# SciML/SciMLSensitivity.jl

Hardware: NVIDIA H100
Metric: ensemble adjoint trajectories/sec (higher is better)
Workload: dtype f64

## Files before the change

include/b200adj.h:

```cpp
#ifndef B200ADJ_H
#define B200ADJ_H
#include <stdint.h>
#ifdef __cplusplus
extern "C" {
#endif

enum {
    B200ADJ_FAM_LV = 0,
    B200ADJ_FAM_LORENZ = 1,
    B200ADJ_FAM_ROBERTSON = 2,
    B200ADJ_FAM_SDE_LV = 3,
    B200ADJ_FAM_MLP = 4,
    B200ADJ_FAM_SDE_LINEAR = 5,
    B200ADJ_FAM_BALL = 6,
    B200ADJ_FAM_RELAX = 7
};
#define B200ADJ_FAM_USER_BASE 100
int32_t b200adj_register_family(const char* plugin_path, int32_t* family_id);
int32_t b200adj_family_info(int32_t family_id, int32_t* d, int32_t* P, const char** name);

enum { B200ADJ_SA_INTERPOLATING = 0, B200ADJ_SA_GAUSS = 1, B200ADJ_SA_QUADRATURE = 2, B200ADJ_SA_BACKSOLVE = 3,
       B200ADJ_SA_GAUSSKRONROD = 4  };
enum { B200ADJ_ST_TSIT5_FIXED = 0, B200ADJ_ST_ROSENBROCK23 = 1, B200ADJ_ST_EM = 2, B200ADJ_ST_EULER_HEUN = 3,
       B200ADJ_ST_TSIT5_ADAPTIVE = 4  };
enum { B200ADJ_F64 = 0, B200ADJ_F32 = 1, B200ADJ_BF16_F32ACC = 2 };
enum { B200ADJ_COST_EXPLICIT = 0, B200ADJ_COST_AFFINE = 1 };

#define B200ADJ_FLAG_NO_START            1u
#define B200ADJ_FLAG_NO_CHECKPOINTING    2u
#define B200ADJ_FLAG_CKPT_EVERY_STEP     4u
#define B200ADJ_FLAG_STORED_NOISE        8u

#define B200ADJ_FLAG_TRACE              16u
#define B200ADJ_FLAG_NO_ROTATE          32u
#define B200ADJ_FLAG_DENSE_FORWARD      64u
#define B200ADJ_FLAG_NCCL_ALLREDUCE    128u
#define B200ADJ_CREATE_FLAGS (B200ADJ_FLAG_STORED_NOISE | B200ADJ_FLAG_TRACE | B200ADJ_FLAG_NO_ROTATE | B200ADJ_FLAG_DENSE_FORWARD | B200ADJ_FLAG_NCCL_ALLREDUCE)

#define B200ADJ_OK                 0
#define B200ADJ_ERR_INVALID       -1
#define B200ADJ_ERR_UNSUPPORTED   -2
#define B200ADJ_ERR_NO_DEVICE     -3
#define B200ADJ_ERR_CUDA          -4
#define B200ADJ_ERR_STATE         -5
#define B200ADJ_ERR_OOM           -6

typedef struct b200adj_cfg {
    int32_t rhs_family, sensealg, stepper, dtype;
    int32_t d, P, m, K;
    int64_t N;
    double  t0, t1, dt;
    double  abstol, reltol;
// ... 74 lines not shown
```

scimlsensitivity.jl_b200/_lib.py:

```python
import ctypes as C
import os
import shutil
import subprocess

_PKG = os.path.dirname(os.path.abspath(__file__))
_ROOT = os.path.dirname(_PKG)
_CSRC = os.path.join(_PKG, "csrc")
LIB_PATH = os.environ.get("B200ADJ_LIB", os.path.join(_PKG, "libb200adj.so"))

FAM = {"lv": 0, "lorenz": 1, "robertson": 2, "sde_lv": 3, "mlp": 4, "sde_linear": 5, "ball": 6, "relax": 7}
SA = {"interpolating": 0, "gauss": 1, "quadrature": 2, "backsolve": 3, "gauss_kronrod": 4}
ST = {"tsit5_fixed": 0, "rosenbrock23": 1, "em": 2, "euler_heun": 3, "tsit5_adaptive": 4}
DTYPE = {"f64": 0, "f32": 1, "bf16_f32acc": 2}
COST = {"explicit": 0, "affine": 1}
FLAG_NO_START, FLAG_NO_CHECKPOINTING, FLAG_CKPT_EVERY_STEP, FLAG_STORED_NOISE, FLAG_TRACE, FLAG_NO_ROTATE, FLAG_DENSE_FORWARD, FLAG_NCCL_ALLREDUCE = 1, 2, 4, 8, 16, 32, 64, 128
ERR = {0: "OK", -1: "INVALID", -2: "UNSUPPORTED", -3: "NO_DEVICE", -4: "CUDA", -5: "STATE", -6: "OOM"}

EXPORTS = ["b200adj_create", "b200adj_forward", "b200adj_reverse", "b200adj_set_reverse_options", "b200adj_set_tolerances", "b200adj_set_continuous_cost", "b200adj_set_cost_family", "b200adj_register_family", "b200adj_family_info", "b200adj_set_events", "b200adj_set_event_param_shift", "b200adj_set_continuous_callback", "b200adj_set_continuous_callback_params", "b200adj_event_times", "b200adj_family_conditions", "b200adj_set_family_events", "b200adj_event_flags", "b200adj_get_noise", "b200adj_set_stream",
           "b200adj_synchronize", "b200adj_launch_count", "b200adj_get_step_counts", "b200adj_get_block_trace", "b200adj_destroy",
           "b200adj_last_error", "b200adj_version", "b200adj_sizeof_cfg",
           "b200adj_comm_unique_id", "b200adj_comm_init", "b200adj_comm_init_all", "b200adj_comm_allreduce", "b200adj_comm_size", "b200adj_comm_is_fused"]


class B200AdjError(RuntimeError):
    def __init__(self, code, msg):
        super().__init__(f"b200adj error {code} ({ERR.get(code, '?')}): {msg}")
        self.code = code


class Cfg(C.Structure):
# ... 339 lines not shown
```

scimlsensitivity.jl_b200/csrc/api.cu:

```cuda
#include <dlfcn.h>

#include "handle.h"

using namespace b200adj;
namespace {

thread_local std::string g_create_error;

const double TSIT5_A[7][6] = {
    {0},
    {0.161},
    {-0.008480655492356989, 0.335480655492357},
    {2.8971530571054935, -6.359448489975075, 4.3622954328695815},
    {5.325864828439257, -11.748883564062828, 7.4955393428898365, -0.09249506636175525},
    {5.86145544294642, -12.92096931784711, 8.159367898576159, -0.071584973281401, -0.028269050394068383},
    {0.09646076681806523, 0.01, 0.4798896504144996, 1.379008574103742, -3.290069515436081, 2.324710524099774}};
const double TSIT5_C[7] = {0.0, 0.161, 0.327, 0.9, 0.9800255409045097, 1.0, 1.0};
const double TSIT5_BT[7] = {-0.00178001105222577714, -0.0008164344596567469, 0.007880878010261995, -0.1447110071732629,
                            0.5823571654525552, -0.45808210592918697, 0.015151515151515152};

std::vector<const FamilyVTable*>& family_registry() { static std::vector<const FamilyVTable*> r; return r; }

template <class F, bool FIXED_GRID, bool ROS, bool F32>
FamilyVTable builtin_family(const char* name) {
// ... 345 lines not shown
        if (block < 32 || block > 512 || (block % 32) != 0) { g_create_error = "block_threads must be a multiple of 32 in [32, 512]"; return B200ADJ_ERR_INVALID; }
        if (mlp) block = MLP_TB;
        if (ckpt_every > 1) {
            if (int32_t rc = support(SR_CKPT)) return rc;
            if (ckpt_every > S) ckpt_every = (int)S;
            const size_t need = (size_t)ckpt_every * d * block * esz(*cfg);
            if (need > 160 * 1024) { g_create_error = "checkpoint_every * d * block_threads * sizeof(real) exceeds 160 KB of shared memory: lower checkpoint_every or block_threads"; return B200ADJ_ERR_INVALID; }
        }
    }

    Handle* h = new Handle();
    h->cfg = *cfg; h->cfg.m = m; h->path = path;
    h->saveat.assign(cfg->saveat, cfg->saveat + cfg->K);
    h->cfg.saveat = h->saveat.data();
    h->S = (int)S; h->maxs = maxs; h->block = block; h->ckpt_every = ckpt_every;
    h->grid = (int)((cfg->N + block - 1) / block);
    h->nsm = nsm; h->qgrid = quad_grid(cfg->N, nsm);
    h->qpartials_blocks = (size_t)h->qgrid + 1;
    h->maxseg = ros ? 2 * maxs : 4096;
#define CREATE_TRY(expr)                                                                         \
    do { cudaError_t _e = (expr); if (_e != cudaSuccess) {                                       \
        g_create_error = std::string(#expr) + ": " + cudaGetErrorString(_e);                     \
        int32_t rc = (_e == cudaErrorMemoryAllocation) ? B200ADJ_ERR_OOM : B200ADJ_ERR_CUDA;     \
        free_all(h); delete h; return rc; } } while (0)
    CREATE_TRY(cudaSetDevice(cfg->device));
    CREATE_TRY(cudaStreamCreateWithFlags(&h->own_stream, cudaStreamNonBlocking));
    h->stream = h->own_stream;
    const size_t N = (size_t)cfg->N, e = esz(*cfg);
    h->fwd_K = cfg->K; h->fwd_saveat = h->saveat;
    CREATE_TRY(upload_table(&h->d_saveat, cfg->saveat, (size_t)cfg->K));
// ... 384 lines not shown
    } else if (h->path == Path::MLP) {
        rc = mlp_forward_dispatch(h, du0, dp, h->fwd_K > 0 ? dsaved : nullptr, dstatus);
    } else if (h->path == Path::FIXED && c.dtype == B200ADJ_F32) {
        OdeFwdArgsT<float> a;
        memset(&a, 0, sizeof(a));
        a.u0 = (const float*)du0; a.p = (const float*)dp; a.ckpt = (float*)h->d_ckpt; a.saved = h->fwd_K > 0 ? (float*)dsaved : nullptr;
        a.save_of_step = h->d_fwd_save_of_step; a.status = dstatus; a.N = c.N; a.Npad = h->Npad; a.S = h->S; a.ckpt_every = h->ckpt_every;
        cast_tables(h->tb, &a.tb);
        rc = launch(vt->fwd_f32, h, a);
    } else if (h->path == Path::FIXED) {
        OdeFwdArgs a;
        memset(&a, 0, sizeof(a));
        a.u0 = du0; a.p = dp; a.ckpt = h->d_ckpt; a.saved = h->fwd_K > 0 ? dsaved : nullptr; a.save_of_step = h->d_fwd_save_of_step;
        a.status = dstatus; a.N = c.N; a.Npad = h->Npad; a.S = h->S; a.tb = h->tb; a.ckpt_every = h->ckpt_every;
        a.event_of_step = h->d_event_of_step; a.ev_s = h->d_ev_s; a.ev_c = h->d_ev_c; a.ev_ps = h->d_ev_ps; a.ev_pc = h->d_ev_pc; a.nev = h->nev;
        rc = launch(vt->fwd, h, a);
    } else {
        SdeFwdArgs a;
        a.u0 = du0; a.p = dp; a.ckpt = h->d_ckpt; a.saved = h->fwd_K > 0 ? dsaved : nullptr; a.save_of_step = h->d_fwd_save_of_step;
        a.status = dstatus; a.N = c.N; a.S = h->S; a.h = c.dt; a.seed = c.seed; a.traj_offset = c.traj_offset;
        a.noise_in = nullptr; a.noise_out = nullptr;
        if (dW_in) {
            CUDA_TRY(h, cudaMemcpyAsync(h->d_noise, dW_in, (size_t)h->S * c.m * N * e,
                                        c.buffers_on_device ? cudaMemcpyDeviceToDevice : cudaMemcpyHostToDevice, h->stream));
            a.noise_in = h->d_noise; h->noise_valid = true;
        } else if (c.flags & B200ADJ_FLAG_STORED_NOISE) {
            a.noise_out = h->d_noise; h->noise_valid = true;
        } else {
            h->noise_valid = false;
        }
// ... 150 lines not shown
```

scimlsensitivity.jl_b200/csrc/disp_fixed.inc:

```
#include "handle.h"
namespace b200adj {
static int balanced_threads(const Handle* h, int slots) {
    const bool no_rotate = (h->cfg.flags & B200ADJ_FLAG_NO_ROTATE) != 0;
    if (!no_rotate && slots > 128 && (slots % 128) != 0) return ((slots + 127) / 128) * 128;
    return slots;
}
template <class Fam>
int launch_fwd(Handle* h, const OdeFwdArgs& a) {
    if (h->nev > 0) {
        if (h->cfg.shared_p) tsit5_forward_kernel<Fam, true, double, true><<<h->grid, h->block, 0, h->stream>>>(a);
        else tsit5_forward_kernel<Fam, false, double, true><<<h->grid, h->block, 0, h->stream>>>(a);
        h->launches++;
        return 0;
    }
    if (h->cfg.shared_p) tsit5_forward_kernel<Fam, true><<<h->grid, h->block, 0, h->stream>>>(a);
    else tsit5_forward_kernel<Fam, false><<<h->grid, h->block, 0, h->stream>>>(a);
    h->launches++;
    return 0;
}
template <class Fam, int SA, bool SHARED_P, int COST, bool CONT, class R>
int launch_rev_seg(Handle* h, const OdeRevArgsT<R>& a, int threads) {
    if constexpr (SA == SA_INTERP || SA == SA_GAUSS) {
        const size_t smem = rev_seg_smem_bytes<Fam::D, R>(h->block, h->ckpt_every);
        if (smem > 30 * 1024 && cudaFuncSetAttribute(tsit5_reverse_kernel<Fam, SA, SHARED_P, COST, CONT, R, true>, cudaFuncAttributeMaxDynamicSharedMemorySize, (int)smem) != cudaSuccess) return B200ADJ_ERR_CUDA;
// ... 44 lines not shown
    a.slots = h->block; a.ckpt_every = h->ckpt_every;
    const int threads = SA == SA_BACKSOLVE ? h->block : balanced_threads(h, h->block);
    if (h->ckpt_every > 1) return h->cont_on ? launch_rev_seg<Fam, SA, SHARED_P, COST, true, double>(h, a, threads)
                                             : launch_rev_seg<Fam, SA, SHARED_P, COST, false, double>(h, a, threads);
    const size_t smem = SA == SA_BACKSOLVE ? 0 : rev_smem_bytes<Fam::D>(h->block);
    if (h->nev > 0) {
        if constexpr (SA == SA_QUAD) return B200ADJ_ERR_UNSUPPORTED;
        else {
            if (h->cont_on) return B200ADJ_ERR_UNSUPPORTED;
            if (smem > 30 * 1024 && cudaFuncSetAttribute(tsit5_reverse_kernel<Fam, SA, SHARED_P, COST, false, double, false, true>, cudaFuncAttributeMaxDynamicSharedMemorySize, (int)smem) != cudaSuccess) return B200ADJ_ERR_CUDA;
            tsit5_reverse_kernel<Fam, SA, SHARED_P, COST, false, double, false, true><<<h->grid, h->block, smem, h->stream>>>(a);
            h->launches++;
            return 0;
        }
    }
    if (h->cont_on) {
        if (smem > 30 * 1024 && cudaFuncSetAttribute(tsit5_reverse_kernel<Fam, SA, SHARED_P, COST, true>, cudaFuncAttributeMaxDynamicSharedMemorySize, (int)smem) != cudaSuccess) return B200ADJ_ERR_CUDA;
        tsit5_reverse_kernel<Fam, SA, SHARED_P, COST, true><<<h->grid, threads, smem, h->stream>>>(a);
    } else {
        if (smem > 30 * 1024 && cudaFuncSetAttribute(tsit5_reverse_kernel<Fam, SA, SHARED_P, COST, false>, cudaFuncAttributeMaxDynamicSharedMemorySize, (int)smem) != cudaSuccess) return B200ADJ_ERR_CUDA;
        tsit5_reverse_kernel<Fam, SA, SHARED_P, COST, false><<<h->grid, threads, smem, h->stream>>>(a);
    }
    h->launches++;
    return 0;
}
template <class Fam, int SA>
int launch_rev_sa(Handle* h, const OdeRevArgs& a) {
    const bool sp = h->cfg.shared_p;
    const bool ex = h->cfg.cost_kind == B200ADJ_COST_EXPLICIT;
    if (sp) return ex ? launch_rev_b<Fam, SA, true, COST_EXPLICIT>(h, a) : launch_rev_b<Fam, SA, true, COST_AFFINE>(h, a);
    return ex ? launch_rev_b<Fam, SA, false, COST_EXPLICIT>(h, a) : launch_rev_b<Fam, SA, false, COST_AFFINE>(h, a);
}
template <class Fam>
int launch_rev(Handle* h, const OdeRevArgs& a) {
    switch (h->cfg.sensealg) {
    case B200ADJ_SA_INTERPOLATING: return launch_rev_sa<Fam, SA_INTERP>(h, a);
    case B200ADJ_SA_GAUSS: return launch_rev_sa<Fam, SA_GAUSS>(h, a);
    case B200ADJ_SA_BACKSOLVE: return launch_rev_sa<Fam, SA_BACKSOLVE>(h, a);
    case B200ADJ_SA_GAUSSKRONROD: return launch_rev_sa<Fam, SA_GK>(h, a);
    case B200ADJ_SA_QUADRATURE: {
        const b200adj_cfg& c = h->cfg;
        int rc = ensure_quad_buffers(h);
        if (rc) return rc;
        OdeRevArgs ar = a; ar.adj_dense = h->d_adj_dense;
        rc = launch_rev_sa<Fam, SA_QUAD>(h, ar);
        if (rc) return rc;
        Tsit5QuadArgs q;
        memset(&q, 0, sizeof(q));
        q.ckpt = h->d_ckpt; q.adj_dense = h->d_adj_dense; q.p = a.p; q.saveat = h->d_saveat;
// ... 17 lines not shown
```

scimlsensitivity.jl_b200/csrc/handle.h:

```cpp
#pragma once
#include <cuda_runtime.h>
#include <math.h>
#include <stdint.h>
#include <stdio.h>
#include <string.h>
#include <stdlib.h>

#include <string>
#include <vector>

#include "../../include/b200adj.h"
#include "ode_tsit5.cuh"
#include "sde_em.cuh"
#include "ros23.cuh"
#include "mlp.cuh"
#include "tsit5_quad.cuh"
#include "mlp_tc.cuh"
#include "mlp_tc_wide.cuh"
#include "tsit5_adaptive.cuh"

namespace b200adj {

enum class Path {
    FIXED,
    T5A,
    ROS,
    SDE,
    MLP
};

struct Handle {
    b200adj_cfg cfg;
    Path path = Path::FIXED;
    std::vector<double> saveat;
    std::vector<int32_t> save_of_step;
    int S = 0;
    int64_t Npad = 0;
    int block = 64, grid = 0, nsm = 132;
    int ckpt_every = 1;
    cudaStream_t stream = nullptr, own_stream = nullptr;
    double* d_ckpt = nullptr;
    double* d_noise = nullptr;
    double* d_partials = nullptr;
    double* d_adj_dense = nullptr;
    unsigned long long* d_trace = nullptr;
    unsigned int* d_ticket = nullptr;
    int32_t* d_save_of_step = nullptr;
    int maxs = 0;
    double adj_abstol = 0, adj_reltol = 0;
    bool cont_on = false;
    double cost_av[4] = {0, 0, 0, 0}, cost_bv[4] = {0, 0, 0, 0}, cont_av[4] = {0, 0, 0, 0}, cont_bv[4] = {0, 0, 0, 0};
    bool has_dgdp = false, has_cdgdp = false;
    double dgdp_c[8] = {0}, dgdp_e[8] = {0}, cdgdp_c[8] = {0}, cdgdp_e[8] = {0};
    float* d_kst = nullptr;
// ... 32 lines not shown
        if (_e != cudaSuccess) {                                                               \
            (h)->err = std::string(#expr) + ": " + cudaGetErrorString(_e);                     \
            return B200ADJ_ERR_CUDA;                                                           \
        }                                                                                      \
    } while (0)

inline bool is_sde(const b200adj_cfg& c) { return c.stepper == B200ADJ_ST_EM || c.stepper == B200ADJ_ST_EULER_HEUN; }
inline bool is_adaptive(const Handle* h) { return h->path == Path::T5A || h->path == Path::ROS; }
inline bool is_fixed_dt(const Handle* h) { return h->path == Path::T5A && h->cfg.stepper == B200ADJ_ST_TSIT5_FIXED; }
inline bool is_mlp_tc(const Handle* h) { return h->path == Path::MLP && h->cfg.dtype == B200ADJ_BF16_F32ACC; }
inline uint32_t kernel_flags(const Handle* h) {
    const uint32_t f = h->cfg.flags;
    return ((f & B200ADJ_FLAG_NO_START) ? KF_NO_START : 0u) | ((f & B200ADJ_FLAG_NO_CHECKPOINTING) ? KF_NO_CHECKPOINTING : 0u) |
           ((f & B200ADJ_FLAG_CKPT_EVERY_STEP) ? KF_CKPT_EVERY_STEP : 0u) | (h->cont_on ? KF_CONT_COST : 0u) |
           (is_fixed_dt(h) ? KF_FIXED_DT : 0u);
}
inline size_t esz(const b200adj_cfg& c) { return c.dtype == B200ADJ_F64 ? sizeof(double) : sizeof(float); }

void tsit5_weights(double th, double* w, double (*Rout)[4] = nullptr);
void build_tsit5_tables(double h, Tsit5Tables* t);
template <class T, class S> inline void cast_tables(const S& src, T* dst) {
    for (int i = 0; i < 7; i++) for (int j = 0; j < 6; j++) dst->hA[i][j] = (float)src.hA[i][j];
    for (int i = 0; i < 4; i++) for (int j = 0; j < 7; j++) dst->hBst[i][j] = (float)src.hBst[i][j];
    for (int i = 0; i < 3; i++) for (int j = 0; j < 7; j++) dst->hBq[i][j] = (float)src.hBq[i][j];
    for (int i = 0; i < 3; i++) dst->hGW[i] = (float)src.hGW[i];
    for (int i = 0; i < 7; i++) for (int j = 0; j < 4; j++) dst->hHm[i][j] = (float)src.hHm[i][j];
    for (int j = 0; j < 7; j++) dst->hR4[j] = (float)src.hR4[j];
}


// ... 50 lines not shown
```

scimlsensitivity.jl_b200/csrc/ode_tsit5.cuh:

```cuda
#pragma once
#include <cuda_runtime.h>
#include <stdint.h>
#include "families.cuh"
#include "quadgk.cuh"

namespace b200adj {

template <class R> struct Tsit5TablesT {
    R hA[7][6];
    R hBst[4][7];
    R hBq[3][7];
    R hGW[3];
    R hHm[7][4];
    R hR4[7];
};
using Tsit5Tables = Tsit5TablesT<double>;

constexpr int P2P_PMAX = 8, P2P_MAXRANKS = 8;
struct P2PComm {
    double* slots[P2P_MAXRANKS];
    unsigned long long* flags[P2P_MAXRANKS];
    int32_t nranks, rank;
    unsigned long long epoch;
};
// ... 90 lines not shown
        R acc = u[i];
#pragma unroll
        for (int j = 0; j < S_; j++) acc = fma(tb.hA[S_][j], k[j][i], acc);
        out[i] = acc;
    }
}
template <int D, class R> __device__ __forceinline__ void tsit5_dense(const R* u, const R (*k)[D], const R* w, R* out) {
#pragma unroll
    for (int i = 0; i < D; i++) {
        R acc = u[i];
#pragma unroll
        for (int j = 0; j < 7; j++) acc = fma(w[j], k[j][i], acc);
        out[i] = acc;
    }
}
template <int D, class R> __device__ __forceinline__ void tsit5_hermite_c4(const Tsit5TablesT<R>& tb, const R (*k)[D], R* c4) {
#pragma unroll
    for (int i = 0; i < D; i++) {
        R acc = tb.hR4[0] * k[0][i];
#pragma unroll
        for (int j = 1; j < 7; j++) acc = fma(tb.hR4[j], k[j][i], acc);
        c4[i] = acc;
    }
}
template <int D, class R>
__device__ __forceinline__ void tsit5_dense_hermite(const R* u, const R* du, const R* k1, const R* k7, const R* c4, const R* w, R* out) {
#pragma unroll
    for (int i = 0; i < D; i++) out[i] = fma(w[3], c4[i], fma(w[2], k7[i], fma(w[1], k1[i], fma(w[0], du[i], u[i]))));
}

__device__ __forceinline__ void named_bar_sync(int id, int nthreads) { asm volatile("bar.sync %0, %1;" ::"r"(id), "r"(nthreads) : "memory"); }
__device__ __forceinline__ void named_bar_arrive(int id, int nthreads) { asm volatile("bar.arrive %0, %1;" ::"r"(id), "r"(nthreads) : "memory"); }

template <int P, class R>
__device__ __forceinline__ void fixed_event_params(const double* ev_ps, const double* ev_pc, int upto, const R* p0, R* p) {
#pragma unroll
    for (int q = 0; q < P; q++) p[q] = p0[q];
    if (!ev_ps) return;
    for (int e = 0; e < upto; e++) {
#pragma unroll
        for (int q = 0; q < P; q++) p[q] = (R)ev_ps[e * P + q] * p[q] + (R)ev_pc[e * P + q];
    }
}

template <class Fam, bool SHARED_P, class R = double, bool EV = false>
__global__ void __launch_bounds__(512) tsit5_forward_kernel(const __grid_constant__ OdeFwdArgsT<R> a) {
    constexpr int D = Fam::D, P = Fam::P;
    const int64_t gi = (int64_t)blockIdx.x * blockDim.x + threadIdx.x;
    const bool active = gi < a.N;
    const int64_t i = active ? gi : a.N - 1;
    R p[P];
#pragma unroll
    for (int q = 0; q < P; q++) p[q] = SHARED_P ? __ldg(a.p + q) : __ldg(a.p + (int64_t)q * a.N + i);
    R u[D], k[7][D], tmp[D];
    load_state<D>(a.u0, a.N, i, u);
    const int64_t stride = (int64_t)D * a.N, cstride = (int64_t)D * a.Npad;
    const int CK = a.ckpt_every > 1 ? a.ckpt_every : 1;
    store_state<D>(a.ckpt, a.Npad, gi, u);
    if (active && a.saved) { int ks = a.save_of_step[0]; if (ks >= 0) store_state<D>(a.saved + (int64_t)ks * stride, a.N, i, u); }
    Fam::f(u, p, k[0]);
// ... 5 lines not shown
        tsit5_stage<D, 5>(a.tb, u, k, tmp); Fam::f(tmp, p, k[5]);
        tsit5_stage<D, 6>(a.tb, u, k, tmp);
#pragma unroll
        for (int j = 0; j < D; j++) u[j] = tmp[j];
        if (EV) {
            const int e = a.event_of_step[n + 1];
            if (e >= 0 && n + 1 < a.S) {
#pragma unroll
                for (int j = 0; j < D; j++) u[j] = (R)a.ev_s[e * D + j] * u[j] + (R)a.ev_c[e * D + j];
                if (a.ev_ps) {
#pragma unroll
                    for (int q = 0; q < P; q++) p[q] = (R)a.ev_ps[e * P + q] * p[q] + (R)a.ev_pc[e * P + q];
                }
            }
        }
        Fam::f(u, p, k[0]);
        if (CK == 1) store_state<D>(a.ckpt + (int64_t)(n + 1) * cstride, a.Npad, gi, u);
        else if ((n + 1) % CK == 0) store_state<D>(a.ckpt + (int64_t)((n + 1) / CK) * cstride, a.Npad, gi, u);
        else if (n + 1 == a.S) store_state<D>(a.ckpt + (int64_t)((a.S + CK - 1) / CK) * cstride, a.Npad, gi, u);
        if (active && a.saved) { int ks = a.save_of_step[n + 1]; if (ks >= 0) store_state<D>(a.saved + (int64_t)ks * stride, a.N, i, u); }
    }
    if (active && a.status) {
        bool ok = true;
#pragma unroll
        for (int j = 0; j < D; j++) ok = ok && isfinite(u[j]);
        a.status[i] = ok ? 0 : 1;
    }
}

__device__ __forceinline__ void st_release_sys(unsigned long long* p, unsigned long long v) { asm volatile("st.release.sys.global.u64 [%0], %1;" ::"l"(p), "l"(v) : "memory"); }
__device__ __forceinline__ unsigned long long ld_acquire_sys(const unsigned long long* p) { unsigned long long v; asm volatile("ld.acquire.sys.global.u64 %0, [%1];" : "=l"(v) : "l"(p) : "memory"); return v; }
__device__ __forceinline__ double ld_relaxed_sys_f64(const double* p) { double v; asm volatile("ld.relaxed.sys.global.f64 %0, [%1];" : "=d"(v) : "l"(p) : "memory"); return v; }

template <int P, class RO>
__device__ __forceinline__ void reduce_dp(const double* acc, double* partials, RO* dp, unsigned int* ticket, const P2PComm* pc = nullptr) {
    __shared__ double s_red[16 * P];
    const int nwarps = (int)(blockDim.x >> 5);
    __shared__ bool s_last;
    const int lane = threadIdx.x & 31, warp = threadIdx.x >> 5;
#pragma unroll
    for (int q = 0; q < P; q++) {
// ... 71 lines not shown
#pragma unroll
        for (int j = 0; j < D; j++) lam[j] += fma(a.cost_a[j], y[j], a.cost_b[j]);
    }
}

#ifndef B200_REV_MAXREG
#define B200_REV_MAXREG 128
#endif
#ifndef REV_CH_DEF
#define REV_CH_DEF 4
#endif
constexpr int REV_CH = REV_CH_DEF, REV_NST = 2;
static_assert(REV_CH_DEF <= 4, "hand-over barrier ids are keyed by step & 3: the block barrier period must not exceed 4 steps");
template <int D, class R = double> constexpr size_t rev_smem_bytes(int block) { return (size_t)REV_NST * REV_CH * D * block * sizeof(R); }
template <int D, class R = double> constexpr size_t rev_seg_smem_bytes(int block, int C) { return (size_t)C * D * block * sizeof(R); }
template <class Fam, int SA, bool SHARED_P, int COST, bool CONT, class R = double, bool SEG = false, bool EV = false>
__global__ void __maxnreg__(B200_REV_MAXREG) tsit5_reverse_kernel(const __grid_constant__ OdeRevArgsT<R> a) {
    constexpr int D = Fam::D, P = Fam::P;
    const int BLOCK = a.slots;
    const bool rot = (int)blockDim.x > BLOCK;
    const int wid = (int)(threadIdx.x >> 5), q4 = (BLOCK >> 7) << 2, rw = (BLOCK >> 5) & 3;
    const bool top = rot && wid >= q4;
    auto group_of = [&](int c) -> int {
        if (!top) return wid;
        const int e = ((wid - q4) - c) & 3;
        return e < rw ? q4 + e : -1;
    };
    int grp = group_of(0);
    auto member_gi = [&]() -> int64_t { return (int64_t)blockIdx.x * BLOCK + grp * 32 + (int)(threadIdx.x & 31); };
    auto member_i = [&]() -> int64_t { const int64_t g = member_gi(); return (grp >= 0 && g < a.N) ? g : a.N - 1; };
    int64_t gi = member_gi();
    bool active = grp >= 0 && gi < a.N;
    int64_t i = active ? gi : a.N - 1;
// ... 80 lines not shown
                    tsit5_stage<D, 5>(tb, ub, kk, tt_); Fam::f(tt_, p, kk[5]);
                    tsit5_stage<D, 6>(tb, ub, kk, y);
                    fsal = false;
                }
            }
        }
    } else {
        R kf[7][D];
        R ka[7][D];
        R ulo[D], uhi[D];
        constexpr int CH = REV_CH, NST = REV_NST;
        extern __shared__ __align__(128) unsigned char s_ck_raw[];
        R* const s_ck = reinterpret_cast<R*>(s_ck_raw);
        __shared__ __align__(8) uint64_t s_bar[NST];
        const uint32_t row_bytes = (uint32_t)(BLOCK * sizeof(R));
        const int NC = (a.S + CH - 1) / CH;
        const R* ck_col = a.ckpt + (int64_t)blockIdx.x * BLOCK;
        auto issue_chunk = [&](int k) {
            const int st = k % NST;
            const int cnt = min(CH, a.S - k * CH);
            mbar_expect_tx(&s_bar[st], (uint32_t)(cnt * D) * row_bytes);
            for (int j = 0; j < cnt; j++) {
                const int nn = a.S - 1 - (k * CH + j);
#pragma unroll
                for (int dd = 0; dd < D; dd++)
                    tma_load_1d(&s_ck[(size_t)((st * CH + j) * D + dd) * BLOCK], ck_col + ((int64_t)nn * D + dd) * Npad, row_bytes, &s_bar[st]);
            }
        };
        if (!SEG) {
            if (threadIdx.x == 0) {
                for (int st = 0; st < NST; st++) mbar_init(&s_bar[st], 1);
                mbar_fence_init();
            }
            __syncthreads();
            if (threadIdx.x == 0) for (int k = 0; k < NST && k < NC; k++) issue_chunk(k);
        }
        const int CK = SEG ? a.ckpt_every : 1;
        const int MROW = SEG ? (a.S + CK - 1) / CK : a.S;
// ... 1 lines not shown
        constexpr int NV = 4 * D + P;
        __shared__ R s_mig[3 * NV * 32];
        __shared__ R s_migp[SHARED_P ? 1 : 3 * P * 32];
        if (!SHARED_P && top && grp >= 0) {
#pragma unroll
            for (int q = 0; q < P; q++) s_migp[((grp - q4) * P + q) * 32 + (threadIdx.x & 31)] = p[q];
        }
        load_state<D>(a.ckpt + (int64_t)MROW * cstride, Npad, grp >= 0 ? gi : 0, uhi);
        {
            int ks = a.save_of_step[a.S];
            if (ks >= 0) add_cotangent<D, COST>(a, ks, stride, N, i, uhi, lam);
            Fam::f(uhi, p, kf[6]);
            Fam::vjp_u(uhi, p, lam, ka[0]);
            add_continuous<D, CONT>(a, uhi, ka[0]);
        }
        bool need_left = false;
        for (int n = a.S - 1; n >= 0; n--) {
            const int c = a.S - 1 - n, k = c / CH, jj = c % CH, st = k % NST;
            if (top) {
                const int lane = (int)(threadIdx.x & 31);
                grp = group_of(c);
                if (c > 0 && grp >= 0) {
                    named_bar_sync(1 + (grp - q4) * 4 + (c & 3), 64);
                    const R* m = s_mig + (size_t)(grp - q4) * NV * 32 + lane;
#pragma unroll
                    for (int j = 0; j < D; j++) { lam[j] = m[j * 32]; ka[0][j] = m[(D + j) * 32]; kf[6][j] = m[(2 * D + j) * 32]; uhi[j] = m[(3 * D + j) * 32]; }
#pragma unroll
                    for (int q = 0; q < P; q++) mu[q] = m[(4 * D + q) * 32];
                    if (!SHARED_P) {
#pragma unroll
                        for (int q = 0; q < P; q++) p[q] = s_migp[((grp - q4) * P + q) * 32 + lane];
                    }
                }
            }
            if (!SEG) {
                if (jj == 0) mbar_wait(&s_bar[st], (uint32_t)((k / NST) & 1));
                if (grp >= 0) {
#pragma unroll
                    for (int dd = 0; dd < D; dd++) ulo[dd] = s_ck[(size_t)((st * CH + jj) * D + dd) * BLOCK + grp * 32 + (threadIdx.x & 31)];
                }
                if (jj == CH - 1 || n == 0) {
                    __syncthreads();
                    if (threadIdx.x == 0 && k + NST < NC) issue_chunk(k + NST);
                }
            } else {
                const int m = n / CK, js = n - m * CK;
                const int slot = grp * 32 + (int)(threadIdx.x & 31);
                if (grp >= 0 && (n == a.S - 1 || js == CK - 1)) {
                    const int cnt = min(CK, a.S - m * CK);
                    R us[D], ts[D];
                    load_state<D>(a.ckpt + (int64_t)m * cstride, Npad, member_gi(), us);
#pragma unroll
                    for (int dd = 0; dd < D; dd++) s_ck[(size_t)dd * BLOCK + slot] = us[dd];
                    Fam::f(us, p, kf[0]);
// ... 6 lines not shown
                        tsit5_stage<D, 6>(tb, us, kf, ts);
#pragma unroll
                        for (int dd = 0; dd < D; dd++) { us[dd] = ts[dd]; s_ck[(size_t)(q * D + dd) * BLOCK + slot] = ts[dd]; }
                        Fam::f(us, p, kf[0]);
                    }
                }
                if (grp >= 0) {
#pragma unroll
                    for (int dd = 0; dd < D; dd++) ulo[dd] = s_ck[(size_t)(js * D + dd) * BLOCK + slot];
                }
                if (jj == CH - 1 || n == 0) __syncthreads();
            }
            if (grp < 0) continue;

            R tmp[D];
            Fam::f(ulo, p, kf[0]);
            tsit5_stage<D, 1>(tb, ulo, kf, tmp); Fam::f(tmp, p, kf[1]);
            tsit5_stage<D, 2>(tb, ulo, kf, tmp); Fam::f(tmp, p, kf[2]);
            tsit5_stage<D, 3>(tb, ulo, kf, tmp); Fam::f(tmp, p, kf[3]);
            tsit5_stage<D, 4>(tb, ulo, kf, tmp); Fam::f(tmp, p, kf[4]);
            tsit5_stage<D, 5>(tb, ulo, kf, tmp); Fam::f(tmp, p, kf[5]);

            if (EV && need_left) {
                tsit5_stage<D, 6>(tb, ulo, kf, uhi);
                Fam::f(uhi, p, kf[6]);
                Fam::vjp_u(uhi, p, lam, ka[0]);
                add_continuous<D, CONT>(a, uhi, ka[0]);
                need_left = false;
            }
            R du[D], c4[D];
            tsit5_hermite_c4<D>(tb, kf, c4);
#pragma unroll
            for (int j = 0; j < D; j++) du[j] = uhi[j] - ulo[j];
#ifdef REV_MIDSYNC
            __syncthreads();
#endif
            R ls[D], y[D], dg[P];
            if (SA == SA_INTERP) {
                Fam::vjp_p(uhi, p, lam, dg);
#pragma unroll
                for (int q = 0; q < P; q++) mu[q] = fma(tb.hA[6][0], dg[q], mu[q]);
            }
#define B200_ADJ_STAGE(S_, YEXPR)                                                          \
            tsit5_stage<D, S_>(tb, lam, ka, ls);                                           \
            YEXPR;                                                                         \
            Fam::vjp_u(y, p, ls, ka[S_]); add_continuous<D, CONT>(a, y, ka[S_]);                 \
// ... 107 lines not shown
```

scimlsensitivity.jl_b200/engine.py:

```python
import numpy as np

from . import _lib
from .problems import FAMILIES, FAMILY_CONDITIONS, AffineCost, ParamAffine, VectorContinuousCallback


def _is_torch(x):
    return hasattr(x, "data_ptr") and hasattr(x, "device")


class DeviceEnsemble:

    def __init__(self, family, sensealg, stepper, N, saveat, tspan, dt, *, shared_p=True, cost=None,
                 on_device=False, device=0, no_start=False, checkpointing=True, ckpt_every_step=False,
                 stored_noise=False, seed=0, traj_offset=0, block_threads=0, abstol=1e-6, reltol=1e-3,
                 quad_abstol=1e-6, quad_reltol=1e-3, dtype="f64", trace=False, max_steps=0, pin_outputs=False,
                 checkpoint_every=1, no_rotate=False, dense_forward=False, nccl_allreduce=False):
        d, P, m = FAMILIES[family]
        cfg = _lib.Cfg()
        cfg.rhs_family, cfg.sensealg, cfg.stepper, cfg.dtype = _lib.FAM[family], _lib.SA[sensealg], _lib.ST[stepper], _lib.DTYPE[dtype]
        cfg.d, cfg.P, cfg.m, cfg.N = d, P, m, int(N)
        cfg.t0, cfg.t1, cfg.dt = float(tspan[0]), float(tspan[1]), float(dt)
        cfg.abstol, cfg.reltol, cfg.quad_abstol, cfg.quad_reltol = abstol, reltol, quad_abstol, quad_reltol
        cfg.shared_p, cfg.buffers_on_device, cfg.device = int(shared_p), int(on_device), int(device)
        if isinstance(cost, AffineCost):
            cfg.cost_kind = _lib.COST["affine"]
            cfg.cost_a, cfg.cost_b = (float(cost.a), float(cost.b)) if cost.is_scalar else (0.0, 0.0)
        else:
            cfg.cost_kind = _lib.COST["explicit"]
        cfg.seed, cfg.traj_offset = int(seed), int(traj_offset)
        cfg.mlp_hidden = 64 if family == "mlp" else 0
        self.dtype = dtype
# ... 5 lines not shown
            flags |= _lib.FLAG_NO_START
        if not checkpointing:
            flags |= _lib.FLAG_NO_CHECKPOINTING
        if ckpt_every_step:
            flags |= _lib.FLAG_CKPT_EVERY_STEP
        if stored_noise:
            flags |= _lib.FLAG_STORED_NOISE
        if trace:
            flags |= _lib.FLAG_TRACE
        if no_rotate:
            flags |= _lib.FLAG_NO_ROTATE
        if dense_forward:
            flags |= _lib.FLAG_DENSE_FORWARD
        if nccl_allreduce:
            flags |= _lib.FLAG_NCCL_ALLREDUCE
        cfg.flags, cfg.block_threads = flags, int(block_threads)
        self.family, self.d, self.P, self.m, self.N, self.K = family, d, P, m, int(N), len(saveat)
        self.shared_p, self.on_device, self.device = bool(shared_p), bool(on_device), int(device)
        self.adaptive = stepper in ("rosenbrock23", "tsit5_adaptive")
        self.events = None
        self.S = 0 if self.adaptive else int(round((cfg.t1 - cfg.t0) / cfg.dt))
        self.saveat = np.ascontiguousarray(saveat, dtype=np.float64)
        self.fwd_saveat, self.fwd_K = self.saveat.copy(), len(self.saveat)
        self.handle = _lib.Handle(cfg, self.saveat)
        if isinstance(cost, AffineCost) and not cost.is_scalar:
            self.handle.set_cost_family(0, np.broadcast_to(np.asarray(cost.a, dtype=np.float64), (d,)), np.broadcast_to(np.asarray(cost.b, dtype=np.float64), (d,)))
        self._keep = []
        self.pin_outputs, self._pinned = bool(pin_outputs), {}
        if self.on_device:
            self.use_current_torch_stream()
# ... 145 lines not shown
```

Baseline: 23.48 million.

## Store paired Hermite coefficients in checkpoints to halve reverse Tsit5 stage recomputation

For fixed-step f64 Interpolating/Gauss adjoints, the forward kernel now stores every other checkpoint slot as the Hermite c4 coefficient instead of the state. The reverse kernel then recomputes the Tsit5 stages once per pair of steps and caches the partner step's c4 and k0 in extra shared memory, roughly halving RHS evaluations in the reverse pass. An unpair kernel restores a plain checkpoint layout when the reverse configuration cannot read the paired form. The costs are more shared memory per block, extra branching and register pressure, and an opt-out flag for the plain layout.

```diff
diff --git a/include/b200adj.h b/include/b200adj.h
--- a/include/b200adj.h
+++ b/include/b200adj.h
@@ -35,7 +35,9 @@
 #define B200ADJ_FLAG_NO_ROTATE          32u
 #define B200ADJ_FLAG_DENSE_FORWARD      64u
 #define B200ADJ_FLAG_NCCL_ALLREDUCE    128u
-#define B200ADJ_CREATE_FLAGS (B200ADJ_FLAG_STORED_NOISE | B200ADJ_FLAG_TRACE | B200ADJ_FLAG_NO_ROTATE | B200ADJ_FLAG_DENSE_FORWARD | B200ADJ_FLAG_NCCL_ALLREDUCE)
+#define B200ADJ_FLAG_PLAIN_CKPT        256u
+#define B200ADJ_CREATE_FLAGS (B200ADJ_FLAG_STORED_NOISE | B200ADJ_FLAG_TRACE | B200ADJ_FLAG_NO_ROTATE | B200ADJ_FLAG_DENSE_FORWARD | B200ADJ_FLAG_NCCL_ALLREDUCE | \
+                              B200ADJ_FLAG_PLAIN_CKPT)
 
 #define B200ADJ_OK                 0
 #define B200ADJ_ERR_INVALID       -1
diff --git a/scimlsensitivity.jl_b200/_lib.py b/scimlsensitivity.jl_b200/_lib.py
--- a/scimlsensitivity.jl_b200/_lib.py
+++ b/scimlsensitivity.jl_b200/_lib.py
@@ -13,7 +13,7 @@
 ST = {"tsit5_fixed": 0, "rosenbrock23": 1, "em": 2, "euler_heun": 3, "tsit5_adaptive": 4}
 DTYPE = {"f64": 0, "f32": 1, "bf16_f32acc": 2}
 COST = {"explicit": 0, "affine": 1}
-FLAG_NO_START, FLAG_NO_CHECKPOINTING, FLAG_CKPT_EVERY_STEP, FLAG_STORED_NOISE, FLAG_TRACE, FLAG_NO_ROTATE, FLAG_DENSE_FORWARD, FLAG_NCCL_ALLREDUCE = 1, 2, 4, 8, 16, 32, 64, 128
+FLAG_NO_START, FLAG_NO_CHECKPOINTING, FLAG_CKPT_EVERY_STEP, FLAG_STORED_NOISE, FLAG_TRACE, FLAG_NO_ROTATE, FLAG_DENSE_FORWARD, FLAG_NCCL_ALLREDUCE, FLAG_PLAIN_CKPT = 1, 2, 4, 8, 16, 32, 64, 128, 256
 ERR = {0: "OK", -1: "INVALID", -2: "UNSUPPORTED", -3: "NO_DEVICE", -4: "CUDA", -5: "STATE", -6: "OOM"}
 
 EXPORTS = ["b200adj_create", "b200adj_forward", "b200adj_reverse", "b200adj_set_reverse_options", "b200adj_set_tolerances", "b200adj_set_continuous_cost", "b200adj_set_cost_family", "b200adj_register_family", "b200adj_family_info", "b200adj_set_events", "b200adj_set_event_param_shift", "b200adj_set_continuous_callback", "b200adj_set_continuous_callback_params", "b200adj_event_times", "b200adj_family_conditions", "b200adj_set_family_events", "b200adj_event_flags", "b200adj_get_noise", "b200adj_set_stream",
diff --git a/scimlsensitivity.jl_b200/csrc/api.cu b/scimlsensitivity.jl_b200/csrc/api.cu
--- a/scimlsensitivity.jl_b200/csrc/api.cu
+++ b/scimlsensitivity.jl_b200/csrc/api.cu
@@ -383,6 +383,7 @@
     h->saveat.assign(cfg->saveat, cfg->saveat + cfg->K);
     h->cfg.saveat = h->saveat.data();
     h->S = (int)S; h->maxs = maxs; h->block = block; h->ckpt_every = ckpt_every;
+    h->paired_ok = path == Path::FIXED && cfg->dtype == B200ADJ_F64 && ckpt_every == 1 && !(cfg->flags & B200ADJ_FLAG_PLAIN_CKPT);
     h->grid = (int)((cfg->N + block - 1) / block);
     h->nsm = nsm; h->qgrid = quad_grid(cfg->N, nsm);
     h->qpartials_blocks = (size_t)h->qgrid + 1;
@@ -797,6 +798,7 @@
         a.u0 = du0; a.p = dp; a.ckpt = h->d_ckpt; a.saved = h->fwd_K > 0 ? dsaved : nullptr; a.save_of_step = h->d_fwd_save_of_step;
         a.status = dstatus; a.N = c.N; a.Npad = h->Npad; a.S = h->S; a.tb = h->tb; a.ckpt_every = h->ckpt_every;
         a.event_of_step = h->d_event_of_step; a.ev_s = h->d_ev_s; a.ev_c = h->d_ev_c; a.ev_ps = h->d_ev_ps; a.ev_pc = h->d_ev_pc; a.nev = h->nev;
+        h->fwd_paired = reads_paired(h);
         rc = launch(vt->fwd, h, a);
     } else {
         SdeFwdArgs a;
diff --git a/scimlsensitivity.jl_b200/csrc/disp_fixed.inc b/scimlsensitivity.jl_b200/csrc/disp_fixed.inc
--- a/scimlsensitivity.jl_b200/csrc/disp_fixed.inc
+++ b/scimlsensitivity.jl_b200/csrc/disp_fixed.inc
@@ -1,3 +1,5 @@
+#include <type_traits>
+
 #include "handle.h"
 namespace b200adj {
 static int balanced_threads(const Handle* h, int slots) {
@@ -5,8 +7,25 @@
     if (!no_rotate && slots > 128 && (slots % 128) != 0) return ((slots + 127) / 128) * 128;
     return slots;
 }
+template <class Fam> constexpr bool paired_built() {
+#ifdef B200ADJ_FAMILY
+    return false;
+#else
+    return !std::is_same<Fam, Robertson>::value;
+#endif
+}
 template <class Fam>
 int launch_fwd(Handle* h, const OdeFwdArgs& a) {
+    if constexpr (paired_built<Fam>()) {
+        if (h->fwd_paired) {
+            if (h->cfg.shared_p) tsit5_forward_kernel<Fam, true, double, false, true><<<h->grid, h->block, 0, h->stream>>>(a);
+            else tsit5_forward_kernel<Fam, false, double, false, true><<<h->grid, h->block, 0, h->stream>>>(a);
+            h->launches++;
+            return 0;
+        }
+    } else {
+        h->fwd_paired = false;
+    }
     if (h->nev > 0) {
         if (h->cfg.shared_p) tsit5_forward_kernel<Fam, true, double, true><<<h->grid, h->block, 0, h->stream>>>(a);
         else tsit5_forward_kernel<Fam, false, double, true><<<h->grid, h->block, 0, h->stream>>>(a);
@@ -82,6 +101,15 @@
             return 0;
         }
     }
+    if constexpr (paired_built<Fam>() && (SA == SA_INTERP || SA == SA_GAUSS)) {
+        if (h->fwd_paired) {
+            const size_t psmem = rev_paired_smem_bytes<Fam::D>(h->block);
+            if (cudaFuncSetAttribute(tsit5_reverse_kernel<Fam, SA, SHARED_P, COST, false, double, false, false, true>, cudaFuncAttributeMaxDynamicSharedMemorySize, (int)psmem) != cudaSuccess) return B200ADJ_ERR_CUDA;
+            tsit5_reverse_kernel<Fam, SA, SHARED_P, COST, false, double, false, false, true><<<h->grid, threads, psmem, h->stream>>>(a);
+            h->launches++;
+            return 0;
+        }
+    }
     if (h->cont_on) {
         if (smem > 30 * 1024 && cudaFuncSetAttribute(tsit5_reverse_kernel<Fam, SA, SHARED_P, COST, true>, cudaFuncAttributeMaxDynamicSharedMemorySize, (int)smem) != cudaSuccess) return B200ADJ_ERR_CUDA;
         tsit5_reverse_kernel<Fam, SA, SHARED_P, COST, true><<<h->grid, threads, smem, h->stream>>>(a);
@@ -101,6 +129,19 @@
 }
 template <class Fam>
 int launch_rev(Handle* h, const OdeRevArgs& a) {
+    if constexpr (paired_built<Fam>()) {
+        if (h->fwd_paired && !reads_paired(h)) {
+            OdeFwdArgs u;
+            memset(&u, 0, sizeof(u));
+            u.ckpt = const_cast<double*>(a.ckpt); u.p = a.p; u.N = a.N; u.Npad = a.Npad; u.S = a.S; u.tb = a.tb;
+            const int pairs = a.S / 2 > 0 ? a.S / 2 : 1;
+            const dim3 grid((unsigned)((a.Npad + 255) / 256), (unsigned)(pairs < 64 ? pairs : 64));
+            if (h->cfg.shared_p) tsit5_unpair_kernel<Fam, true><<<grid, 256, 0, h->stream>>>(u);
+            else tsit5_unpair_kernel<Fam, false><<<grid, 256, 0, h->stream>>>(u);
+            h->launches++;
+            h->fwd_paired = false;
+        }
+    }
     switch (h->cfg.sensealg) {
     case B200ADJ_SA_INTERPOLATING: return launch_rev_sa<Fam, SA_INTERP>(h, a);
     case B200ADJ_SA_GAUSS: return launch_rev_sa<Fam, SA_GAUSS>(h, a);
diff --git a/scimlsensitivity.jl_b200/csrc/handle.h b/scimlsensitivity.jl_b200/csrc/handle.h
--- a/scimlsensitivity.jl_b200/csrc/handle.h
+++ b/scimlsensitivity.jl_b200/csrc/handle.h
@@ -38,6 +38,7 @@
     int64_t Npad = 0;
     int block = 64, grid = 0, nsm = 132;
     int ckpt_every = 1;
+    bool paired_ok = false, fwd_paired = false;
     cudaStream_t stream = nullptr, own_stream = nullptr;
     double* d_ckpt = nullptr;
     double* d_noise = nullptr;
@@ -100,6 +101,9 @@
     return ((f & B200ADJ_FLAG_NO_START) ? KF_NO_START : 0u) | ((f & B200ADJ_FLAG_NO_CHECKPOINTING) ? KF_NO_CHECKPOINTING : 0u) |
            ((f & B200ADJ_FLAG_CKPT_EVERY_STEP) ? KF_CKPT_EVERY_STEP : 0u) | (h->cont_on ? KF_CONT_COST : 0u) |
            (is_fixed_dt(h) ? KF_FIXED_DT : 0u);
+}
+inline bool reads_paired(const Handle* h) {
+    return h->paired_ok && (h->cfg.sensealg == B200ADJ_SA_INTERPOLATING || h->cfg.sensealg == B200ADJ_SA_GAUSS) && h->nev == 0 && !h->cont_on;
 }
 inline size_t esz(const b200adj_cfg& c) { return c.dtype == B200ADJ_F64 ? sizeof(double) : sizeof(float); }
 
diff --git a/scimlsensitivity.jl_b200/csrc/ode_tsit5.cuh b/scimlsensitivity.jl_b200/csrc/ode_tsit5.cuh
--- a/scimlsensitivity.jl_b200/csrc/ode_tsit5.cuh
+++ b/scimlsensitivity.jl_b200/csrc/ode_tsit5.cuh
@@ -128,13 +128,13 @@
         out[i] = acc;
     }
 }
-template <int D, class R> __device__ __forceinline__ void tsit5_hermite_c4(const Tsit5TablesT<R>& tb, const R (*k)[D], R* c4) {
+template <int D, class R> __device__ __forceinline__ void tsit5_hermite_c4(const Tsit5TablesT<R>& tb, const R (*k)[D], const R* k7, R* c4) {
 #pragma unroll
     for (int i = 0; i < D; i++) {
         R acc = tb.hR4[0] * k[0][i];
 #pragma unroll
-        for (int j = 1; j < 7; j++) acc = fma(tb.hR4[j], k[j][i], acc);
-        c4[i] = acc;
+        for (int j = 1; j < 6; j++) acc = fma(tb.hR4[j], k[j][i], acc);
+        c4[i] = fma(tb.hR4[6], k7[i], acc);
     }
 }
 template <int D, class R>
@@ -157,7 +157,7 @@
     }
 }
 
-template <class Fam, bool SHARED_P, class R = double, bool EV = false>
+template <class Fam, bool SHARED_P, class R = double, bool EV = false, bool PAIRED = false>
 __global__ void __launch_bounds__(512) tsit5_forward_kernel(const __grid_constant__ OdeFwdArgsT<R> a) {
     constexpr int D = Fam::D, P = Fam::P;
     const int64_t gi = (int64_t)blockIdx.x * blockDim.x + threadIdx.x;
@@ -193,10 +193,22 @@
                 }
             }
         }
-        Fam::f(u, p, k[0]);
-        if (CK == 1) store_state<D>(a.ckpt + (int64_t)(n + 1) * cstride, a.Npad, gi, u);
-        else if ((n + 1) % CK == 0) store_state<D>(a.ckpt + (int64_t)((n + 1) / CK) * cstride, a.Npad, gi, u);
-        else if (n + 1 == a.S) store_state<D>(a.ckpt + (int64_t)((a.S + CK - 1) / CK) * cstride, a.Npad, gi, u);
+        if (PAIRED) {
+            Fam::f(u, p, k[6]);
+            if (n & 1) {
+                R c4[D];
+                tsit5_hermite_c4<D>(a.tb, k, k[6], c4);
+                store_state<D>(a.ckpt + (int64_t)n * cstride, a.Npad, gi, c4);
+            }
+#pragma unroll
+            for (int j = 0; j < D; j++) k[0][j] = k[6][j];
+            if (!((n + 1) & 1) || n + 1 == a.S) store_state<D>(a.ckpt + (int64_t)(n + 1) * cstride, a.Npad, gi, u);
+        } else {
+            Fam::f(u, p, k[0]);
+            if (CK == 1) store_state<D>(a.ckpt + (int64_t)(n + 1) * cstride, a.Npad, gi, u);
+            else if ((n + 1) % CK == 0) store_state<D>(a.ckpt + (int64_t)((n + 1) / CK) * cstride, a.Npad, gi, u);
+            else if (n + 1 == a.S) store_state<D>(a.ckpt + (int64_t)((a.S + CK - 1) / CK) * cstride, a.Npad, gi, u);
+        }
         if (active && a.saved) { int ks = a.save_of_step[n + 1]; if (ks >= 0) store_state<D>(a.saved + (int64_t)ks * stride, a.N, i, u); }
     }
     if (active && a.status) {
@@ -204,6 +216,28 @@
 #pragma unroll
         for (int j = 0; j < D; j++) ok = ok && isfinite(u[j]);
         a.status[i] = ok ? 0 : 1;
+    }
+}
+
+template <class Fam, bool SHARED_P>
+__global__ void __launch_bounds__(256) tsit5_unpair_kernel(const __grid_constant__ OdeFwdArgs a) {
+    constexpr int D = Fam::D, P = Fam::P;
+    const int64_t gi = (int64_t)blockIdx.x * blockDim.x + threadIdx.x;
+    if (gi >= a.Npad) return;
+    const int64_t i = gi < a.N ? gi : a.N - 1, cstride = (int64_t)D * a.Npad;
+    double p[P], u[D], k[6][D], tmp[D];
+#pragma unroll
+    for (int q = 0; q < P; q++) p[q] = SHARED_P ? __ldg(a.p + q) : __ldg(a.p + (int64_t)q * a.N + i);
+    for (int m = blockIdx.y; 2 * m + 1 < a.S; m += gridDim.y) {
+        load_state<D>(a.ckpt + (int64_t)(2 * m) * cstride, a.Npad, gi, u);
+        Fam::f(u, p, k[0]);
+        tsit5_stage<D, 1>(a.tb, u, k, tmp); Fam::f(tmp, p, k[1]);
+        tsit5_stage<D, 2>(a.tb, u, k, tmp); Fam::f(tmp, p, k[2]);
+        tsit5_stage<D, 3>(a.tb, u, k, tmp); Fam::f(tmp, p, k[3]);
+        tsit5_stage<D, 4>(a.tb, u, k, tmp); Fam::f(tmp, p, k[4]);
+        tsit5_stage<D, 5>(a.tb, u, k, tmp); Fam::f(tmp, p, k[5]);
+        tsit5_stage<D, 6>(a.tb, u, k, tmp);
+        store_state<D>(a.ckpt + (int64_t)(2 * m + 1) * cstride, a.Npad, gi, tmp);
     }
 }
 
@@ -305,9 +339,11 @@
 static_assert(REV_CH_DEF <= 4, "hand-over barrier ids are keyed by step & 3: the block barrier period must not exceed 4 steps");
 template <int D, class R = double> constexpr size_t rev_smem_bytes(int block) { return (size_t)REV_NST * REV_CH * D * block * sizeof(R); }
 template <int D, class R = double> constexpr size_t rev_seg_smem_bytes(int block, int C) { return (size_t)C * D * block * sizeof(R); }
-template <class Fam, int SA, bool SHARED_P, int COST, bool CONT, class R = double, bool SEG = false, bool EV = false>
+template <int D, class R = double> constexpr size_t rev_paired_smem_bytes(int block) { return rev_smem_bytes<D, R>(block) + (size_t)2 * D * block * sizeof(R); }
+template <class Fam, int SA, bool SHARED_P, int COST, bool CONT, class R = double, bool SEG = false, bool EV = false, bool PAIRED = false>
 __global__ void __maxnreg__(B200_REV_MAXREG) tsit5_reverse_kernel(const __grid_constant__ OdeRevArgsT<R> a) {
     constexpr int D = Fam::D, P = Fam::P;
+    static_assert(!PAIRED || (!SEG && !EV && !CONT && (SA == SA_INTERP || SA == SA_GAUSS)), "the paired layout serves the plain Interpolating / Gauss step");
     const int BLOCK = a.slots;
     const bool rot = (int)blockDim.x > BLOCK;
     const int wid = (int)(threadIdx.x >> 5), q4 = (BLOCK >> 7) << 2, rw = (BLOCK >> 5) & 3;
@@ -418,14 +454,16 @@
         R* const s_ck = reinterpret_cast<R*>(s_ck_raw);
         __shared__ __align__(8) uint64_t s_bar[NST];
         const uint32_t row_bytes = (uint32_t)(BLOCK * sizeof(R));
-        const int NC = (a.S + CH - 1) / CH;
+        const int off = PAIRED ? (a.S & 1) : 0;
+        const int NC = (a.S + off + CH - 1) / CH;
         const R* ck_col = a.ckpt + (int64_t)blockIdx.x * BLOCK;
         auto issue_chunk = [&](int k) {
             const int st = k % NST;
-            const int cnt = min(CH, a.S - k * CH);
-            mbar_expect_tx(&s_bar[st], (uint32_t)(cnt * D) * row_bytes);
-            for (int j = 0; j < cnt; j++) {
-                const int nn = a.S - 1 - (k * CH + j);
+            const int c0 = k * CH - off, j0 = (PAIRED && c0 < 0) ? -c0 : 0;
+            const int cnt = min(CH, a.S - c0);
+            mbar_expect_tx(&s_bar[st], (uint32_t)((cnt - j0) * D) * row_bytes);
+            for (int j = j0; j < cnt; j++) {
+                const int nn = a.S - 1 - (c0 + j);
 #pragma unroll
                 for (int dd = 0; dd < D; dd++)
                     tma_load_1d(&s_ck[(size_t)((st * CH + j) * D + dd) * BLOCK], ck_col + ((int64_t)nn * D + dd) * Npad, row_bytes, &s_bar[st]);
@@ -457,9 +495,10 @@
             Fam::vjp_u(uhi, p, lam, ka[0]);
             add_continuous<D, CONT>(a, uhi, ka[0]);
         }
+        R* const s_pair = s_ck + (size_t)NST * CH * D * BLOCK;
         bool need_left = false;
         for (int n = a.S - 1; n >= 0; n--) {
-            const int c = a.S - 1 - n, k = c / CH, jj = c % CH, st = k % NST;
+            const int c = a.S - 1 - n, k = (c + off) / CH, jj = (c + off) % CH, st = k % NST;
             if (top) {
                 const int lane = (int)(threadIdx.x & 31);
                 grp = group_of(c);
@@ -476,11 +515,20 @@
                     }
                 }
             }
+            R c4[D], ub[D];
             if (!SEG) {
-                if (jj == 0) mbar_wait(&s_bar[st], (uint32_t)((k / NST) & 1));
+                if (jj == 0 || (PAIRED && c == 0)) mbar_wait(&s_bar[st], (uint32_t)((k / NST) & 1));
                 if (grp >= 0) {
-#pragma unroll
-                    for (int dd = 0; dd < D; dd++) ulo[dd] = s_ck[(size_t)((st * CH + jj) * D + dd) * BLOCK + grp * 32 + (threadIdx.x & 31)];
+                    if (PAIRED && (n & 1)) {
+#pragma unroll
+                        for (int dd = 0; dd < D; dd++) {
+                            c4[dd] = s_ck[(size_t)((st * CH + jj) * D + dd) * BLOCK + grp * 32 + (threadIdx.x & 31)];
+                            ub[dd] = s_ck[(size_t)((st * CH + jj + 1) * D + dd) * BLOCK + grp * 32 + (threadIdx.x & 31)];
+                        }
+                    } else {
+#pragma unroll
+                        for (int dd = 0; dd < D; dd++) ulo[dd] = s_ck[(size_t)((st * CH + jj) * D + dd) * BLOCK + grp * 32 + (threadIdx.x & 31)];
+                    }
                 }
                 if (jj == CH - 1 || n == 0) {
                     __syncthreads();
@@ -517,22 +565,45 @@
             if (grp < 0) continue;
 
             R tmp[D];
-            Fam::f(ulo, p, kf[0]);
-            tsit5_stage<D, 1>(tb, ulo, kf, tmp); Fam::f(tmp, p, kf[1]);
-            tsit5_stage<D, 2>(tb, ulo, kf, tmp); Fam::f(tmp, p, kf[2]);
-            tsit5_stage<D, 3>(tb, ulo, kf, tmp); Fam::f(tmp, p, kf[3]);
-            tsit5_stage<D, 4>(tb, ulo, kf, tmp); Fam::f(tmp, p, kf[4]);
-            tsit5_stage<D, 5>(tb, ulo, kf, tmp); Fam::f(tmp, p, kf[5]);
-
-            if (EV && need_left) {
-                tsit5_stage<D, 6>(tb, ulo, kf, uhi);
-                Fam::f(uhi, p, kf[6]);
-                Fam::vjp_u(uhi, p, lam, ka[0]);
-                add_continuous<D, CONT>(a, uhi, ka[0]);
-                need_left = false;
-            }
-            R du[D], c4[D];
-            tsit5_hermite_c4<D>(tb, kf, c4);
+            const int pslot = grp * 32 + (int)(threadIdx.x & 31);
+            if (!PAIRED || (n == a.S - 1 && !(n & 1))) {
+                Fam::f(ulo, p, kf[0]);
+                tsit5_stage<D, 1>(tb, ulo, kf, tmp); Fam::f(tmp, p, kf[1]);
+                tsit5_stage<D, 2>(tb, ulo, kf, tmp); Fam::f(tmp, p, kf[2]);
+                tsit5_stage<D, 3>(tb, ulo, kf, tmp); Fam::f(tmp, p, kf[3]);
+                tsit5_stage<D, 4>(tb, ulo, kf, tmp); Fam::f(tmp, p, kf[4]);
+                tsit5_stage<D, 5>(tb, ulo, kf, tmp); Fam::f(tmp, p, kf[5]);
+
+                if (EV && need_left) {
+                    tsit5_stage<D, 6>(tb, ulo, kf, uhi);
+                    Fam::f(uhi, p, kf[6]);
+                    Fam::vjp_u(uhi, p, lam, ka[0]);
+                    add_continuous<D, CONT>(a, uhi, ka[0]);
+                    need_left = false;
+                }
+                tsit5_hermite_c4<D>(tb, kf, kf[6], c4);
+            } else if (n & 1) {
+                Fam::f(ub, p, kf[0]);
+                tsit5_stage<D, 1>(tb, ub, kf, tmp); Fam::f(tmp, p, kf[1]);
+                tsit5_stage<D, 2>(tb, ub, kf, tmp); Fam::f(tmp, p, kf[2]);
+                tsit5_stage<D, 3>(tb, ub, kf, tmp); Fam::f(tmp, p, kf[3]);
+                tsit5_stage<D, 4>(tb, ub, kf, tmp); Fam::f(tmp, p, kf[4]);
+                tsit5_stage<D, 5>(tb, ub, kf, tmp); Fam::f(tmp, p, kf[5]);
+                tsit5_stage<D, 6>(tb, ub, kf, ulo);
+                Fam::f(ulo, p, tmp);
+                R c4m[D];
+                tsit5_hermite_c4<D>(tb, kf, tmp, c4m);
+#pragma unroll
+                for (int j = 0; j < D; j++) {
+                    s_pair[(size_t)j * BLOCK + pslot] = c4m[j];
+                    s_pair[(size_t)(D + j) * BLOCK + pslot] = kf[0][j];
+                    kf[0][j] = tmp[j];
+                }
+            } else {
+#pragma unroll
+                for (int j = 0; j < D; j++) { c4[j] = s_pair[(size_t)j * BLOCK + pslot]; kf[0][j] = s_pair[(size_t)(D + j) * BLOCK + pslot]; }
+            }
+            R du[D];
 #pragma unroll
             for (int j = 0; j < D; j++) du[j] = uhi[j] - ulo[j];
 #ifdef REV_MIDSYNC
diff --git a/scimlsensitivity.jl_b200/engine.py b/scimlsensitivity.jl_b200/engine.py
--- a/scimlsensitivity.jl_b200/engine.py
+++ b/scimlsensitivity.jl_b200/engine.py
@@ -14,7 +14,7 @@
                  on_device=False, device=0, no_start=False, checkpointing=True, ckpt_every_step=False,
                  stored_noise=False, seed=0, traj_offset=0, block_threads=0, abstol=1e-6, reltol=1e-3,
                  quad_abstol=1e-6, quad_reltol=1e-3, dtype="f64", trace=False, max_steps=0, pin_outputs=False,
-                 checkpoint_every=1, no_rotate=False, dense_forward=False, nccl_allreduce=False):
+                 checkpoint_every=1, no_rotate=False, dense_forward=False, nccl_allreduce=False, plain_ckpt=False):
         d, P, m = FAMILIES[family]
         cfg = _lib.Cfg()
         cfg.rhs_family, cfg.sensealg, cfg.stepper, cfg.dtype = _lib.FAM[family], _lib.SA[sensealg], _lib.ST[stepper], _lib.DTYPE[dtype]
@@ -50,6 +50,8 @@
             flags |= _lib.FLAG_DENSE_FORWARD
         if nccl_allreduce:
             flags |= _lib.FLAG_NCCL_ALLREDUCE
+        if plain_ckpt:
+            flags |= _lib.FLAG_PLAIN_CKPT
         cfg.flags, cfg.block_threads = flags, int(block_threads)
         self.family, self.d, self.P, self.m, self.N, self.K = family, d, P, m, int(N), len(saveat)
         self.shared_p, self.on_device, self.device = bool(shared_p), bool(on_device), int(device)
```

New measurement: 23.52 million, median of 6. About the same (+0.2%).
